# SmartBFT-Go/consensus

Measured on NVIDIA H100. Metric: ECDSA-P256 verifies/sec at batch=64K, higher is better.
Workload: dtype u32 limbs (integer)

## Files before the change

consensus_b200/csrc/inst_common.cuh:

```cuda
#pragma once
#include "keygroup.cuh"
#include "ops.h"
#include <cstdlib>

namespace sbv {

template <class C> struct Cfg;
template <> struct Cfg<P256> { static constexpr int COZ_MINB = 6, KT_MINB = 7, KT_VARIANT = 2, COMB_MINB = 6; static constexpr bool COMB_INL = true; };
template <> struct Cfg<P384> { static constexpr int COZ_MINB = 4, KT_MINB = 4, KT_VARIANT = 0; };

template <class C>
cudaError_t op_gtable_init(uint32_t *gtab, cudaStream_t st) {
    const size_t entries = (size_t)C::GWINS << C::GW;
    k_gtable_init<C><<<(unsigned)((entries + 127) / 128), 128, 0, st>>>(gtab);
    return cudaGetLastError();
}

template <class C>
cudaError_t op_prep(uint32_t n, const uint8_t *r, const uint8_t *s, const uint8_t *dig, uint32_t dlen, uint32_t *uw, uint8_t *flags,
                    cudaStream_t st) {
    return launch_prep<C, 8>(n, r, s, dig, dlen, uw, flags, st);
}

template <class C>
cudaError_t op_group(uint32_t n, const uint8_t *qx, const uint8_t *qy, uint32_t seed, uint32_t hmask, uint32_t *htab, uint32_t *rep,
                     uint32_t *kcnt, uint32_t threshold, uint32_t max_keys, int32_t *keyid, uint32_t *keylist, int32_t *item_kid,
                     uint32_t *klist, uint32_t *glist, uint32_t *counters, int route, cudaStream_t st) {
    const unsigned blocks = (n + 255) / 256;
    k_kg_insert<C><<<blocks, 256, 0, st>>>(n, qx, qy, seed, hmask, htab, rep, kcnt);
    k_kg_assign<<<blocks, 256, 0, st>>>(n, rep, kcnt, threshold, max_keys, keyid, keylist, counters);
    if (route) k_kg_route<<<blocks, 256, 0, st>>>(n, rep, keyid, item_kid, klist, glist, counters);
    return cudaGetLastError();
}

[[maybe_unused]] static cudaError_t op_route(uint32_t n, const uint32_t *rep, const int32_t *keyid, int32_t *item_kid, uint32_t *klist, uint32_t *glist,
                            uint32_t *counters, cudaStream_t st) {
    k_kg_route<<<(n + 255) / 256, 256, 0, st>>>(n, rep, keyid, item_kid, klist, glist, counters);
    return cudaGetLastError();
}

template <class C>
cudaError_t op_gpart(uint32_t n, const uint32_t *uw, const uint32_t *gtab, uint32_t *gacc, cudaStream_t st) {
    constexpr int BLOCK = 64;
    k_gpart<C, BLOCK, Cfg<C>::KT_MINB - 1><<<(n + BLOCK - 1) / BLOCK, BLOCK, 0, st>>>(n, uw, reinterpret_cast<const uint4 *>(gtab), gacc);
    return cudaGetLastError();
}

template <class C>
cudaError_t op_coz(uint32_t n, const uint8_t *qx, const uint8_t *qy, const uint8_t *r, const uint32_t *uw, const uint8_t *flags,
                   const uint32_t *gtab, uint32_t *tscr, uint8_t *ok, const uint32_t *list, const uint32_t *count, cudaStream_t st) {
    constexpr int BLOCK = 64;
    const size_t smem = (size_t)7 * 2 * C::N * 4 * BLOCK;
    k_verify_coz<C, BLOCK, Cfg<C>::COZ_MINB><<<(n + BLOCK - 1) / BLOCK, BLOCK, smem, st>>>(
        n, qx, qy, r, uw, flags, reinterpret_cast<const uint4 *>(gtab), tscr, ok, list, count);
    return cudaGetLastError();
}

template <class C, int W>
cudaError_t op_kt_build(const uint32_t *nkeys_ptr, uint32_t cap, const uint32_t *keylist, const uint8_t *qx, const uint8_t *qy,
                        uint32_t *bases, uint32_t *hs, uint32_t *ztop, uint32_t *pref, uint32_t *ktab, uint8_t *keyflags, cudaStream_t st) {
    using KT = KeyTab<32 * C::N, W>;
    const unsigned kb = (cap + 63) / 64;
    const unsigned wb = (unsigned)(((size_t)cap * KT::NWIN + 63) / 64);
    static const int bases_variant = getenv("SBV_KT_BASES") ? atoi(getenv("SBV_KT_BASES")) : 0;
    if (bases_variant == 2) k_kt_bases<C, KT, false><<<kb, 64, 0, st>>>(nkeys_ptr, cap, keylist, qx, qy, bases, keyflags);
    else if (bases_variant == 1) k_kt_bases<C, KT, true><<<kb, 64, 0, st>>>(nkeys_ptr, cap, keylist, qx, qy, bases, keyflags);
    else k_kt_bases4<C, KT><<<(unsigned)(((size_t)cap * 4 + 127) / 128), 128, 0, st>>>(nkeys_ptr, cap, keylist, qx, qy, bases, keyflags);
    k_kt_fill<C, W><<<wb, 64, 0, st>>>(nkeys_ptr, cap, bases, keyflags, hs, ztop, ktab);
    k_kt_inv<C, KT><<<kb, 64, 0, st>>>(nkeys_ptr, cap, keyflags, ztop, pref);
    k_kt_final<C, KT><<<wb, 64, 0, st>>>(nkeys_ptr, cap, bases, keyflags, hs, ztop, ktab);
    return cudaGetLastError();
}

template <class C, int W>
cudaError_t op_kt_verify(int reg, int warp, uint32_t n, const uint32_t *slot, const int32_t *kidmap, uint32_t n_slots,
                         const uint8_t *keyflags, const uint8_t *r, const uint32_t *uw, const uint8_t *flags, const uint32_t *gtab,
                         const uint32_t *ktab, uint8_t *ok, const uint32_t *list, const uint32_t *count, const uint32_t *gacc, cudaStream_t st) {
    constexpr int BLOCK = 64, MINB = Cfg<C>::KT_MINB;
    static const int variant = getenv("SBV_KT_VARIANT") ? atoi(getenv("SBV_KT_VARIANT")) : Cfg<C>::KT_VARIANT;
    const uint4 *g4 = reinterpret_cast<const uint4 *>(gtab), *k4 = reinterpret_cast<const uint4 *>(ktab);
    const unsigned blocks = (n + BLOCK - 1) / BLOCK;
#define SBV_KT_ARGS n, slot, kidmap, n_slots, keyflags, r, uw, flags, g4, k4, ok, list, count, gacc
    if (warp) {
        k_verify_kt_warp<C, W><<<(unsigned)(((size_t)n * 32 + 127) / 128), 128, 0, st>>>(n, slot, kidmap, n_slots, keyflags, r, uw, flags, g4, k4, ok);
    } else if (reg) {
        if (variant == 1) k_verify_kt<C, W, BLOCK, MINB, true, true><<<blocks, BLOCK, 0, st>>>(SBV_KT_ARGS);
        else if (variant == 2) k_verify_kt<C, W, BLOCK, MINB - 1, true, true><<<blocks, BLOCK, 0, st>>>(SBV_KT_ARGS);
        else k_verify_kt<C, W, BLOCK, MINB, true, false><<<blocks, BLOCK, 0, st>>>(SBV_KT_ARGS);
    } else {
        if (variant == 1) k_verify_kt<C, W, BLOCK, MINB, false, true><<<blocks, BLOCK, 0, st>>>(SBV_KT_ARGS);
        else if (variant == 2) k_verify_kt<C, W, BLOCK, MINB - 1, false, true><<<blocks, BLOCK, 0, st>>>(SBV_KT_ARGS);
        else k_verify_kt<C, W, BLOCK, MINB, false, false><<<blocks, BLOCK, 0, st>>>(SBV_KT_ARGS);
    }
#undef SBV_KT_ARGS
    return cudaGetLastError();
}

template <class C>
cudaError_t op_comb_build(const uint32_t *nkeys_ptr, uint32_t cap, const uint32_t *keylist, const uint8_t *qx, const uint8_t *qy,
                          uint32_t *bases, uint32_t *hs, uint32_t *ztop, uint32_t *pref, uint32_t *ktab, uint8_t *keyflags, cudaStream_t st) {
    using CT = CombTab<C>;
    const unsigned kb = (cap + 63) / 64;
    const unsigned cb = (unsigned)(((size_t)cap * CT::NCHAIN + 63) / 64);
    k_kt_bases4<C, CT><<<(unsigned)(((size_t)cap * 4 + 127) / 128), 128, 0, st>>>(nkeys_ptr, cap, keylist, qx, qy, bases, keyflags);
    k_comb_affine<C><<<kb, 64, 0, st>>>(nkeys_ptr, cap, keyflags, bases, pref);
    k_comb_fill<C><<<cb, 64, 0, st>>>(nkeys_ptr, cap, bases, keyflags, hs, ztop, ktab);
    k_kt_inv<C, CT><<<kb, 64, 0, st>>>(nkeys_ptr, cap, keyflags, ztop, pref);
    k_kt_final<C, CT><<<cb, 64, 0, st>>>(nkeys_ptr, cap, bases, keyflags, hs, ztop, ktab);
    return cudaGetLastError();
}

template <class C>
cudaError_t op_comb_verify(int reg, int warp, uint32_t n, const uint32_t *slot, const int32_t *kidmap, uint32_t n_slots,
                           const uint8_t *keyflags, const uint8_t *r, const uint32_t *uw, const uint8_t *flags, const uint32_t *gtab,
                           const uint32_t *ktab, uint8_t *ok, const uint32_t *list, const uint32_t *count, const uint32_t *gacc, cudaStream_t st) {
    constexpr int BLOCK = 64;
    (void)slot; (void)n_slots;
    if (reg || warp || !list || !count) return cudaErrorInvalidValue;
    k_verify_comb<C, BLOCK, Cfg<C>::COMB_MINB, Cfg<C>::COMB_INL><<<(n + BLOCK - 1) / BLOCK, BLOCK, 0, st>>>(
        n, kidmap, keyflags, r, uw, flags, reinterpret_cast<const uint4 *>(gtab), reinterpret_cast<const uint4 *>(ktab), ok, list, count, gacc);
    return cudaGetLastError();
}

template <class C, class KT>
constexpr KtGeom kt_geom() {
    using KS = KtSizes<C, KT>;
    return KtGeom{KS::bases_words(1), KS::hs_words(1), KS::ztop_words(1), KS::ktab_words(1)};
}

}
```

consensus_b200/csrc/keygroup.cuh:

```cuda
#pragma once
#include "kernels.cuh"

namespace sbv {

constexpr uint32_t KG_EMPTY = 0xffffffffu;

template <class C>
SBV_DEV uint32_t kg_hash(const uint8_t *__restrict__ qx_be, const uint8_t *__restrict__ qy_be, uint32_t i, uint32_t seed) {
    const uint32_t *x = reinterpret_cast<const uint32_t *>(qx_be + (size_t)i * C::BYTES);
    const uint32_t *y = reinterpret_cast<const uint32_t *>(qy_be + (size_t)i * C::BYTES);
    uint32_t h = seed;
#pragma unroll
    for (int k = 0; k < C::N; k += 2) {
        h = (h ^ __ldg(x + k)) * 0x9E3779B1u;
        h = (h ^ __ldg(y + k + 1)) * 0x85EBCA77u;
        h ^= h >> 15;
    }
    return h;
}
template <class C>
SBV_DEV bool kg_same_key(const uint8_t *__restrict__ qx_be, const uint8_t *__restrict__ qy_be, uint32_t i, uint32_t j) {
    const uint32_t *xi = reinterpret_cast<const uint32_t *>(qx_be + (size_t)i * C::BYTES);
    const uint32_t *xj = reinterpret_cast<const uint32_t *>(qx_be + (size_t)j * C::BYTES);
    const uint32_t *yi = reinterpret_cast<const uint32_t *>(qy_be + (size_t)i * C::BYTES);
    const uint32_t *yj = reinterpret_cast<const uint32_t *>(qy_be + (size_t)j * C::BYTES);
    uint32_t diff = 0;
#pragma unroll
    for (int k = 0; k < C::N; k++) diff |= (__ldg(xi + k) ^ __ldg(xj + k)) | (__ldg(yi + k) ^ __ldg(yj + k));
    return diff == 0;
}

template <class C>
__global__ void __launch_bounds__(256) k_kg_insert(uint32_t n, const uint8_t *__restrict__ qx_be, const uint8_t *__restrict__ qy_be,
                                                   uint32_t seed, uint32_t hmask, uint32_t *__restrict__ htab,
                                                   uint32_t *__restrict__ rep, uint32_t *__restrict__ kcnt) {
    const uint32_t i = blockIdx.x * blockDim.x + threadIdx.x;
    if (i >= n) return;
    uint32_t h = kg_hash<C>(qx_be, qy_be, i, seed) & hmask;
    uint32_t r;
    for (;;) {
        uint32_t cur = htab[h];
        if (cur == KG_EMPTY) {
            cur = atomicCAS(htab + h, KG_EMPTY, i);
            if (cur == KG_EMPTY) { r = i; break; }
        }
        if (kg_same_key<C>(qx_be, qy_be, i, cur)) { r = cur; break; }
        h = (h + 1) & hmask;
    }
    rep[i] = r;
#if defined(__CUDA_ARCH__)
    const uint32_t peers = __match_any_sync(__activemask(), r);
    if ((threadIdx.x & 31) == (uint32_t)(__ffs((int)peers) - 1)) atomicAdd(kcnt + r, (uint32_t)__popc(peers));
#else
    atomicAdd(kcnt + r, 1u);
#endif
}

static __global__ void __launch_bounds__(256) k_kg_assign(uint32_t n, const uint32_t *__restrict__ rep, const uint32_t *__restrict__ kcnt,
                                                   uint32_t threshold, uint32_t max_keys, int32_t *__restrict__ keyid,
                                                   uint32_t *__restrict__ keylist, uint32_t *__restrict__ counters) {
    const uint32_t i = blockIdx.x * blockDim.x + threadIdx.x;
    if (i >= n) return;
    int32_t id = -1;
    if (rep[i] == i && kcnt[i] >= threshold) {
        const uint32_t k = atomicAdd(counters + 0, 1u);
        if (k < max_keys) { id = (int32_t)k; keylist[k] = i; }
    }
    keyid[i] = id;
}

static __global__ void __launch_bounds__(256) k_kg_route(uint32_t n, const uint32_t *__restrict__ rep, const int32_t *__restrict__ keyid,
                                                  int32_t *__restrict__ item_kid, uint32_t *__restrict__ klist, uint32_t *__restrict__ glist,
                                                  uint32_t *__restrict__ counters) {
    const uint32_t i = blockIdx.x * blockDim.x + threadIdx.x;
    const bool live = i < n;
    const int32_t kid = live ? keyid[rep[i]] : -1;
    if (live) item_kid[i] = kid;
#if defined(__CUDA_ARCH__)
    const uint32_t lane = threadIdx.x & 31;
    const uint32_t mk = __ballot_sync(0xffffffffu, live && kid >= 0), mg = __ballot_sync(0xffffffffu, live && kid < 0);
    uint32_t bk = 0, bg = 0;
    if (lane == 0) {
        if (mk) bk = atomicAdd(counters + 1, (uint32_t)__popc(mk));
        if (mg) bg = atomicAdd(counters + 2, (uint32_t)__popc(mg));
    }
    bk = __shfl_sync(0xffffffffu, bk, 0);
    bg = __shfl_sync(0xffffffffu, bg, 0);
    const uint32_t below = (1u << lane) - 1u;
    if (live && kid >= 0) klist[bk + __popc(mk & below)] = i;
    if (live && kid < 0) glist[bg + __popc(mg & below)] = i;
#else
    if (live && kid >= 0) klist[atomicAdd(counters + 1, 1u)] = i;
    if (live && kid < 0) glist[atomicAdd(counters + 2, 1u)] = i;
#endif
}


template <class C, class KT, bool INL>
__global__ void __launch_bounds__(64) k_kt_bases(const uint32_t *__restrict__ nkeys_ptr, uint32_t cap, const uint32_t *__restrict__ keylist,
                                                 const uint8_t *__restrict__ qx_be, const uint8_t *__restrict__ qy_be,
                                                 uint32_t *__restrict__ bases, uint8_t *__restrict__ keyflags) {
    constexpr int N = C::N;
    const uint32_t k = blockIdx.x * blockDim.x + threadIdx.x;
    uint32_t nkeys = __ldg(nkeys_ptr);
    if (nkeys > cap) nkeys = cap;
    if (k >= nkeys) return;
    const uint32_t item = keylist ? keylist[k] : k;
    using A = typename PickArith<C, INL>::type;
    Jac<A> B;
    const bool good = load_key<C>(B.X, B.Y, qx_be, qy_be, item);
    keyflags[k] = good ? 1 : 0;
    if (!good) return;
    C::get_one(B.Z);
#pragma unroll 1
    for (int win = 0; win < KT::NBASE; win++) {
        if (win) {
#pragma unroll 1
            for (int d = 0; d < KT::STEP; d++) pt_double<A>(B);
        }
        uint32_t *o = bases + (size_t)win * 3 * N * cap + k;
#pragma unroll
        for (int i = 0; i < N; i++) { o[(size_t)i * cap] = B.X[i]; o[(size_t)(N + i) * cap] = B.Y[i]; o[(size_t)(2 * N + i) * cap] = B.Z[i]; }
    }
}

template <class C, class KT>
__global__ void __launch_bounds__(128) k_kt_bases4(const uint32_t *__restrict__ nkeys_ptr, uint32_t cap, const uint32_t *__restrict__ keylist,
                                                   const uint8_t *__restrict__ qx_be, const uint8_t *__restrict__ qy_be,
                                                   uint32_t *__restrict__ bases, uint8_t *__restrict__ keyflags) {
    constexpr int N = C::N;
    const uint32_t gt = blockIdx.x * blockDim.x + threadIdx.x;
    const uint32_t k = gt >> 2, role = gt & 3;
    uint32_t nkeys = __ldg(nkeys_ptr);
    if (nkeys > cap) nkeys = cap;
    if (k >= nkeys) return;
    const unsigned qbase = (threadIdx.x & 31) & ~3u, qmask = 0xFu << qbase;
    const uint32_t item = keylist ? keylist[k] : k;
    uint32_t X[N], Y[N], Z[N];
    const bool good = load_key<C>(X, Y, qx_be, qy_be, item);
    if (role == 0) keyflags[k] = good ? 1 : 0;
    if (!good) return;
    C::get_one(Z);
    auto bcast = [&](uint32_t (&v)[N], unsigned src) {
#pragma unroll
        for (int i = 0; i < N; i++) v[i] = __shfl_sync(qmask, v[i], qbase + src);
    };
#pragma unroll 1
    for (int win = 0; win < KT::NBASE; win++) {
        if (win) {
#pragma unroll 1
            for (int d = 0; d < KT::STEP; d++) {
                uint32_t s[N], a[N], b[N], r1[N], r2[N], r3[N], r4[N], t1[N], t2[N];
                C::fadd(s, Y, Y);
                mp_select<N>(a, role == 1 || role == 2, s, Z);
                mp_select<N>(b, role == 1, s, Z);
                C::fmul(r1, a, b);
                uint32_t bb[N];
                mp_copy<N>(bb, r1);
                bcast(bb, 1);
                C::fsub(t1, X, r1);
                C::fadd(t2, X, r1);
                mp_select<N>(a, role == 0, t1, X);
                mp_select<N>(a, role == 2, bb, a);
                mp_select<N>(b, role == 0, t2, bb);
                C::fmul(r2, a, b);
                uint32_t alpha[N], half[N], beta4[N];
                C::fadd(t1, r2, r2);
                C::fadd(alpha, t1, r2);
                C::fhalf(half, r2);
                C::fmul(r3, alpha, alpha);
                mp_copy<N>(beta4, r2);
                bcast(beta4, 1);
                bcast(half, 2);
                uint32_t x3[N], y3[N];
                C::fadd(t1, beta4, beta4);
                C::fsub(x3, r3, t1);
                C::fsub(t2, beta4, x3);
                C::fmul(r4, alpha, t2);
                C::fsub(y3, r4, half);
                mp_copy<N>(X, x3); bcast(X, 0);
                mp_copy<N>(Y, y3); bcast(Y, 0);
                mp_copy<N>(Z, r1); bcast(Z, 2);
            }
        }
        if (role == 0) {
            uint32_t *o = bases + (size_t)win * 3 * N * cap + k;
#pragma unroll
            for (int i = 0; i < N; i++) { o[(size_t)i * cap] = X[i]; o[(size_t)(N + i) * cap] = Y[i]; o[(size_t)(2 * N + i) * cap] = Z[i]; }
        }
    }
}

template <class C>
SBV_DEV void zaddu(uint32_t (&X1)[C::N], uint32_t (&Y1)[C::N], const uint32_t (&X2)[C::N], const uint32_t (&Y2)[C::N],
                   uint32_t (&X3)[C::N], uint32_t (&Y3)[C::N], uint32_t (&h)[C::N]) {
    constexpr int N = C::N;
    uint32_t c[N], w1[N], w2[N], dy[N], d[N], a1[N], t[N];
    C::fsub(h, X1, X2);
    C::fsqr(c, h);
    C::fmul(w1, X1, c);
    C::fmul(w2, X2, c);
    C::fsub(dy, Y1, Y2);
    C::fsqr(d, dy);
    C::fsub(t, w1, w2);
    C::fmul(a1, Y1, t);
    C::fsub(X3, d, w1);
    C::fsub(X3, X3, w2);
    C::fsub(t, w1, X3);
    C::fmul(Y3, dy, t);
    C::fsub(Y3, Y3, a1);
    mp_copy<N>(X1, w1);
    mp_copy<N>(Y1, a1);
}

template <class C, int W>
__global__ void __launch_bounds__(64) k_kt_fill(const uint32_t *__restrict__ nkeys_ptr, uint32_t cap, const uint32_t *__restrict__ bases,
                                                const uint8_t *__restrict__ keyflags, uint32_t *__restrict__ hs,
                                                uint32_t *__restrict__ ztop, uint32_t *__restrict__ ktab) {
    constexpr int N = C::N;
    using KT = KeyTab<32 * N, W>;
    const uint32_t t = blockIdx.x * blockDim.x + threadIdx.x;
    uint32_t nkeys = __ldg(nkeys_ptr);
    if (nkeys > cap) nkeys = cap;
    if (t >= nkeys * KT::NWIN) return;
    const uint32_t k = t % nkeys, win = t / nkeys;
    if (!keyflags[k]) return;
    uint32_t bx[N], by[N], bz[N];
    {
        const uint32_t *o = bases + (size_t)win * 3 * N * cap + k;
#pragma unroll
        for (int i = 0; i < N; i++) { bx[i] = o[(size_t)i * cap]; by[i] = o[(size_t)(N + i) * cap]; bz[i] = o[(size_t)(2 * N + i) * cap]; }
    }
    uint32_t *out = ktab + ((size_t)k * KT::NWIN + win) * KT::ENT * 2 * N;
#pragma unroll
    for (int i = 0; i < N; i++) { out[i] = bx[i]; out[N + i] = by[i]; }
    Jac<C> P;
    mp_copy<N>(P.X, bx); mp_copy<N>(P.Y, by); mp_copy<N>(P.Z, bz);
    uint32_t h[N], h2[N], h3[N];
    C::fadd(h, by, by);
    pt_double<C>(P);
    C::fsqr(h2, h);
    C::fmul(h3, h2, h);
    C::fmul(bx, bx, h2);
    C::fmul(by, by, h3);
    uint32_t zacc[N];
    mp_copy<N>(zacc, P.Z);
    {
        uint32_t *hp = hs + ((size_t)win * (KT::ENT - 1) + 0) * N * cap + k;
#pragma unroll
        for (int i = 0; i < N; i++) { out[2 * N + i] = P.X[i]; out[3 * N + i] = P.Y[i]; hp[(size_t)i * cap] = h[i]; }
    }
    uint32_t px[N], py[N];
    mp_copy<N>(px, P.X); mp_copy<N>(py, P.Y);
#pragma unroll 1
    for (int e = 3; e <= KT::ENT; e++) {
        uint32_t x3[N], y3[N];
        zaddu<C>(bx, by, px, py, x3, y3, h);
        C::fmul(zacc, zacc, h);
        mp_copy<N>(px, x3); mp_copy<N>(py, y3);
        uint32_t *hp = hs + ((size_t)win * (KT::ENT - 1) + (e - 2)) * N * cap + k;
        uint32_t *oe = out + (size_t)(e - 1) * 2 * N;
#pragma unroll
        for (int i = 0; i < N; i++) { oe[i] = px[i]; oe[N + i] = py[i]; hp[(size_t)i * cap] = h[i]; }
    }
    uint32_t *zp = ztop + (size_t)win * N * cap + k;
#pragma unroll
    for (int i = 0; i < N; i++) zp[(size_t)i * cap] = zacc[i];
}

template <class C, class KT>
__global__ void __launch_bounds__(64) k_kt_inv(const uint32_t *__restrict__ nkeys_ptr, uint32_t cap, const uint8_t *__restrict__ keyflags,
                                               uint32_t *__restrict__ ztop, uint32_t *__restrict__ pref) {
    constexpr int N = C::N;
    const uint32_t k = blockIdx.x * blockDim.x + threadIdx.x;
    uint32_t nkeys = __ldg(nkeys_ptr);
    if (nkeys > cap) nkeys = cap;
    if (k >= nkeys || !keyflags[k]) return;
    uint32_t run[N];
    C::get_one(run);
#pragma unroll 1
    for (int win = 0; win < KT::NCHAIN; win++) {
        uint32_t z[N];
        const uint32_t *zp = ztop + (size_t)win * N * cap + k;
        uint32_t *pp = pref + (size_t)win * N * cap + k;
#pragma unroll
        for (int i = 0; i < N; i++) { z[i] = zp[(size_t)i * cap]; pp[(size_t)i * cap] = run[i]; }
        C::fmul(run, run, z);
    }
    uint32_t inv[N];
    p_inv<C>(inv, run);
#pragma unroll 1
    for (int win = KT::NCHAIN - 1; win >= 0; win--) {
        uint32_t z[N], pv[N], zi[N];
        uint32_t *zp = ztop + (size_t)win * N * cap + k;
        const uint32_t *pp = pref + (size_t)win * N * cap + k;
#pragma unroll
        for (int i = 0; i < N; i++) { z[i] = zp[(size_t)i * cap]; pv[i] = pp[(size_t)i * cap]; }
        C::fmul(zi, inv, pv);
        C::fmul(inv, inv, z);
#pragma unroll
        for (int i = 0; i < N; i++) zp[(size_t)i * cap] = zi[i];
    }
}

template <class C, class KT>
__global__ void __launch_bounds__(64) k_kt_final(const uint32_t *__restrict__ nkeys_ptr, uint32_t cap, const uint32_t *__restrict__ bases,
                                                 const uint8_t *__restrict__ keyflags, const uint32_t *__restrict__ hs,
                                                 const uint32_t *__restrict__ ztop, uint32_t *__restrict__ ktab) {
    constexpr int N = C::N;
    const uint32_t t = blockIdx.x * blockDim.x + threadIdx.x;
    uint32_t nkeys = __ldg(nkeys_ptr);
    if (nkeys > cap) nkeys = cap;
    if (t >= nkeys * KT::NCHAIN) return;
    const uint32_t k = t % nkeys, win = t / nkeys;
    if (!keyflags[k]) return;
    uint32_t zi[N];
    {
        const uint32_t *zp = ztop + (size_t)win * N * cap + k;
#pragma unroll
        for (int i = 0; i < N; i++) zi[i] = zp[(size_t)i * cap];
    }
    uint32_t *out = ktab + ((size_t)k * KT::NCHAIN + win) * KT::ENT * 2 * N;
    uint32_t x[N], y[N], h[N];
    {
        const uint32_t *oe = out + (size_t)(KT::ENT - 1) * 2 * N;
#pragma unroll
        for (int i = 0; i < N; i++) { x[i] = oe[i]; y[i] = oe[N + i]; }
    }
#pragma unroll 1
    for (int e = KT::ENT; e >= 1; e--) {
        uint32_t nx[N], ny[N], nh[N];
        if (e >= 2) {
            const uint32_t *on = out + (size_t)(e - 2) * 2 * N;
            const uint32_t *hp = hs + ((size_t)win * (KT::ENT - 1) + (e - 2)) * N * cap + k;
#pragma unroll
            for (int i = 0; i < N; i++) { nx[i] = on[i]; ny[i] = on[N + i]; nh[i] = hp[(size_t)i * cap]; }
        }
        uint32_t *oe = out + (size_t)(e - 1) * 2 * N;
        uint32_t z2[N], z3[N];
        C::fsqr(z2, zi);
        C::fmul(z3, z2, zi);
        C::fmul(x, x, z2);
        C::fmul(y, y, z3);
#pragma unroll
        for (int i = 0; i < N; i++) { oe[i] = x[i]; oe[N + i] = y[i]; }
        if (e >= 2) {
            mp_copy<N>(h, nh);
            C::fmul(zi, zi, h);
            mp_copy<N>(x, nx); mp_copy<N>(y, ny);
        }
    }
    (void)bases;
}


template <class C>
__global__ void __launch_bounds__(64) k_comb_affine(const uint32_t *__restrict__ nkeys_ptr, uint32_t cap, const uint8_t *__restrict__ keyflags,
                                                    uint32_t *__restrict__ bases, uint32_t *__restrict__ pref) {
    constexpr int N = C::N;
    using CT = CombTab<C>;
    const uint32_t k = blockIdx.x * blockDim.x + threadIdx.x;
    uint32_t nkeys = __ldg(nkeys_ptr);
    if (nkeys > cap) nkeys = cap;
    if (k >= nkeys || !keyflags[k]) return;
    uint32_t run[N];
    C::get_one(run);
#pragma unroll 1
    for (int c = 0; c < CT::NBASE; c++) {
        uint32_t z[N];
        const uint32_t *zp = bases + ((size_t)c * 3 + 2) * N * cap + k;
        uint32_t *pp = pref + (size_t)c * N * cap + k;
#pragma unroll
        for (int i = 0; i < N; i++) { z[i] = zp[(size_t)i * cap]; pp[(size_t)i * cap] = run[i]; }
        C::fmul(run, run, z);
    }
    uint32_t inv[N];
    p_inv<C>(inv, run);
#pragma unroll 1
    for (int c = CT::NBASE - 1; c >= 0; c--) {
        uint32_t *o = bases + (size_t)c * 3 * N * cap + k;
        const uint32_t *pp = pref + (size_t)c * N * cap + k;
        uint32_t x[N], y[N], z[N], pv[N], zi[N], z2[N], z3[N];
#pragma unroll
        for (int i = 0; i < N; i++) { x[i] = o[(size_t)i * cap]; y[i] = o[(size_t)(N + i) * cap]; z[i] = o[(size_t)(2 * N + i) * cap]; pv[i] = pp[(size_t)i * cap]; }
        C::fmul(zi, inv, pv);
        C::fmul(inv, inv, z);
        C::fsqr(z2, zi);
        C::fmul(z3, z2, zi);
        C::fmul(x, x, z2);
        C::fmul(y, y, z3);
#pragma unroll
        for (int i = 0; i < N; i++) { o[(size_t)i * cap] = x[i]; o[(size_t)(N + i) * cap] = y[i]; }
    }
}

template <class C>
__global__ void __launch_bounds__(64) k_comb_fill(const uint32_t *__restrict__ nkeys_ptr, uint32_t cap, const uint32_t *__restrict__ bases,
                                                  const uint8_t *__restrict__ keyflags, uint32_t *__restrict__ hs,
                                                  uint32_t *__restrict__ ztop, uint32_t *__restrict__ ktab) {
    constexpr int N = C::N;
    using CT = CombTab<C>;
    const uint32_t t = blockIdx.x * blockDim.x + threadIdx.x;
    uint32_t nkeys = __ldg(nkeys_ptr);
    if (nkeys > cap) nkeys = cap;
    if (t >= nkeys * CT::NCHAIN) return;
    const uint32_t k = t % nkeys, ch = t / nkeys;
    if (!keyflags[k]) return;
    const int b = (int)(ch >> 4), hi = (int)(ch & 15);
    auto base = [&](int c, uint32_t (&x)[N], uint32_t (&y)[N]) {
        const uint32_t *o = bases + (size_t)c * 3 * N * cap + k;
#pragma unroll
        for (int i = 0; i < N; i++) { x[i] = o[(size_t)i * cap]; y[i] = o[(size_t)(N + i) * cap]; }
    };
    uint32_t *out = ktab + ((size_t)k * CT::NCHAIN + ch) * CT::ENT * 2 * N;
    auto store = [&](int slot, const uint32_t (&x)[N], const uint32_t (&y)[N], const uint32_t (&h)[N]) {
        uint32_t *o = out + (size_t)slot * 2 * N;
#pragma unroll
        for (int i = 0; i < N; i++) { o[i] = x[i]; o[N + i] = y[i]; }
        if (slot) {
            uint32_t *hp = hs + ((size_t)ch * (CT::ENT - 1) + (slot - 1)) * N * cap + k;
#pragma unroll
            for (int i = 0; i < N; i++) hp[(size_t)i * cap] = h[i];
        }
    };
    Jac<C> P;
    uint32_t x[N], y[N], h[N];
    C::get_one(P.Z);
    C::get_one(h);
    int first;
    if (hi == 0) {
        uint32_t zero[N];
#pragma unroll
        for (int i = 0; i < N; i++) zero[i] = 0;
        store(0, zero, zero, h);
        base(CT::TEETH * b, P.X, P.Y);
        store(1, P.X, P.Y, h);
        first = 2;
    } else {
        bool empty = true;
#pragma unroll 1
        for (int i = 0; i < 4; i++) {
            if (!((hi >> i) & 1)) continue;
            base(CT::TEETH * b + 4 + i, x, y);
            if (empty) { mp_copy<N>(P.X, x); mp_copy<N>(P.Y, y); empty = false; }
            else pt_madd_table<C>(P, x, y, h);
        }
        store(0, P.X, P.Y, h);
        first = 1;
    }
#pragma unroll 1
    for (int kk = first; kk < CT::ENT; kk++) {
        const int tooth = __ffs(kk) - 1;
        base(CT::TEETH * b + tooth, x, y);
        if (!(((kk ^ (kk >> 1)) >> tooth) & 1)) {
            uint32_t zero[N];
#pragma unroll
            for (int i = 0; i < N; i++) zero[i] = 0;
            C::fsub(y, zero, y);
        }
        pt_madd_table<C>(P, x, y, h);
        store(kk, P.X, P.Y, h);
    }
    uint32_t *zp = ztop + (size_t)ch * N * cap + k;
#pragma unroll
    for (int i = 0; i < N; i++) zp[(size_t)i * cap] = P.Z[i];
}

template <class C, class KT_>
struct KtSizes {
    using KT = KT_;
    static constexpr size_t bases_words(size_t cap) { return (size_t)KT::NBASE * 3 * C::N * cap; }
    static constexpr size_t hs_words(size_t cap) { return (size_t)KT::NCHAIN * (KT::ENT - 1) * C::N * cap; }
    static constexpr size_t ztop_words(size_t cap) { return (size_t)KT::NCHAIN * C::N * cap; }
    static constexpr size_t ktab_words(size_t cap) { return KT::POINTS * 2 * C::N * cap; }
};

}
```

consensus_b200/csrc/pipeline.cu:

```cuda
#include "engine.h"

namespace {

int take_scratch(sbv_engine *e, Dev &d, const CurveOps &ops, const KtOps *kt, size_t n, size_t kcap, cudaStream_t st, Dev::Scratch **out) {
    int idx = (int)(d.ws_next++ % SBV_SCRATCH);
    for (int tries = 0; tries < SBV_SCRATCH && d.ws[idx].open; tries++) idx = (int)(d.ws_next++ % SBV_SCRATCH);
    if (d.ws[idx].open) return sbv_fail(e, SBV_ERR_ARG, "no free scratch set (more launches held open than lanes?)");
    Dev::Scratch &w = d.ws[idx];
    Dev::Scratch::Caps &c = w.caps;
    if (!w.done) {
        for (int j = 0; j < SBV_SCRATCH; j++) {
            Dev::Scratch &x = d.ws[j];
            if (x.done) continue;
            CU(e, cudaEventCreateWithFlags(&x.done, cudaEventDisableTiming));
            CU(e, cudaEventCreateWithFlags(&x.ev_group, cudaEventDisableTiming));
            CU(e, cudaEventCreateWithFlags(&x.ev_prep, cudaEventDisableTiming));
            CU(e, cudaEventCreateWithFlags(&x.ev_tab, cudaEventDisableTiming));
            CU(e, cudaEventCreateWithFlags(&x.ev_gen, cudaEventDisableTiming));
            if (e->tab_hi) {
                int lo_p = 0, hi_p = 0;
                CU(e, cudaDeviceGetStreamPriorityRange(&lo_p, &hi_p));
                CU(e, cudaStreamCreateWithPriority(&x.s_tab, cudaStreamNonBlocking, hi_p));
            } else {
                CU(e, cudaStreamCreateWithFlags(&x.s_tab, cudaStreamNonBlocking));
            }
            CU(e, cudaStreamCreateWithFlags(&x.s_gen, cudaStreamNonBlocking));
        }
    }
    const size_t N = (size_t)ops.N;
    uint32_t hsize = 1;
    while (hsize < 2 * n) hsize <<= 1;
    struct Need { void **p; size_t *cap; size_t need, alloc; };
    const size_t ni = n + n / 8 + 1024, kc = kcap + kcap / 8 + 16;
    uint32_t hs2 = 1;
    while (hs2 < 2 * ni) hs2 <<= 1;
    const bool g = kcap > 0, t = g && kt;
    const KtGeom z{};
    const KtGeom &q = t ? kt->geom : z;
    Need needs[] = {
        {(void **)&w.uw, &c.uw, 2 * N * n * 4, 2 * N * ni * 4},
        {(void **)&w.flags, &c.flags, n, ni},
        {(void **)&w.tscr, &c.tscr, 12 * N * n * 4, 12 * N * ni * 4},
        {(void **)&w.gacc, &c.gacc, g ? 3 * N * n * 4 : 0, 3 * N * ni * 4},
        {(void **)&w.htab, &c.htab, g ? (size_t)hsize * 4 : 0, (size_t)hs2 * 4},
        {(void **)&w.rep, &c.rep, g ? n * 4 : 0, ni * 4},
        {(void **)&w.klist, &c.klist, g ? n * 4 : 0, ni * 4},
        {(void **)&w.glist, &c.glist, g ? n * 4 : 0, ni * 4},
        {(void **)&w.zeroed, &c.zeroed, g ? (n + 4 + 4 * SBV_MAX_CHUNKS) * 4 : 0, (ni + 4 + 4 * SBV_MAX_CHUNKS) * 4},
        {(void **)&w.keyid, &c.keyid, g ? n * 4 : 0, ni * 4},
        {(void **)&w.item_kid, &c.item_kid, g ? n * 4 : 0, ni * 4},
        {(void **)&w.keylist, &c.keylist, t ? kcap * 4 : 0, kc * 4},
        {(void **)&w.keyflags, &c.keyflags, t ? kcap : 0, kc},
        {(void **)&w.bases, &c.bases, q.bases_words * kcap * 4, q.bases_words * kc * 4},
        {(void **)&w.hs, &c.hs, q.hs_words * kcap * 4, q.hs_words * kc * 4},
        {(void **)&w.ztop, &c.ztop, q.ztop_words * kcap * 4, q.ztop_words * kc * 4},
        {(void **)&w.pref, &c.pref, q.ztop_words * kcap * 4, q.ztop_words * kc * 4},
        {(void **)&w.ktab, &c.ktab, q.ktab_words * kcap * 4, q.ktab_words * kc * 4},
    };
    bool grows = false;
    for (const Need &nd : needs) grows = grows || nd.need > *nd.cap;
    if (grows) {
        for (int j = 0; j < SBV_SCRATCH; j++) {
            Dev::Scratch &x = d.ws[j];
            if (x.open && &x != &w) continue;
            if (x.used && x.done) CU(e, cudaEventSynchronize(x.done));
            Dev::Scratch::Caps &cx = x.caps;
            struct Slot { void **p; size_t *cap; };
            const Slot slots[] = {
                {(void **)&x.uw, &cx.uw}, {(void **)&x.flags, &cx.flags}, {(void **)&x.tscr, &cx.tscr}, {(void **)&x.gacc, &cx.gacc},
                {(void **)&x.htab, &cx.htab}, {(void **)&x.rep, &cx.rep}, {(void **)&x.klist, &cx.klist}, {(void **)&x.glist, &cx.glist},
                {(void **)&x.zeroed, &cx.zeroed}, {(void **)&x.keyid, &cx.keyid}, {(void **)&x.item_kid, &cx.item_kid}, {(void **)&x.keylist, &cx.keylist},
                {(void **)&x.keyflags, &cx.keyflags}, {(void **)&x.bases, &cx.bases}, {(void **)&x.hs, &cx.hs}, {(void **)&x.ztop, &cx.ztop},
                {(void **)&x.pref, &cx.pref}, {(void **)&x.ktab, &cx.ktab},
            };
            static_assert(sizeof(slots) / sizeof(slots[0]) == sizeof(needs) / sizeof(needs[0]), "one slot per buffer");
            for (size_t q = 0; q < sizeof(slots) / sizeof(slots[0]); q++) {
                if (needs[q].need <= *slots[q].cap) continue;
                if (*slots[q].p) cudaFree(*slots[q].p);
                *slots[q].p = nullptr;
                *slots[q].cap = 0;
                CU(e, cudaMalloc(slots[q].p, needs[q].alloc));
                *slots[q].cap = needs[q].alloc;
            }
        }
    }
    w.hsize = hsize;
    if (w.used) CU(e, cudaStreamWaitEvent(st, w.done, 0));
    w.used = true;
    *out = &w;
    return 0;
}

cudaEvent_t *prof_take(sbv_engine *e, Dev &d) {
    if (!e->profiling) return nullptr;
    if (d.prof_used + 5 > d.prof_events.size()) {
        size_t old = d.prof_events.size();
        d.prof_events.resize(old + 128);
        for (size_t i = old; i < d.prof_events.size(); i++)
            if (cudaEventCreate(&d.prof_events[i]) != cudaSuccess) { d.prof_events.resize(i); return nullptr; }
    }
    cudaEvent_t *ev = &d.prof_events[d.prof_used];
    d.prof_used += 5;
    return ev;
}

}

void sbv_scratch_free(Dev &d) {
    for (auto &w : d.ws) {
        void *ptrs[] = {w.uw, w.flags, w.tscr, w.gacc, w.htab, w.rep, w.keylist, w.klist, w.glist, w.zeroed, w.keyid, w.item_kid, w.bases, w.hs, w.ztop, w.pref, w.ktab, w.keyflags};
        for (void *p : ptrs) if (p) cudaFree(p);
        cudaEvent_t evs[] = {w.done, w.ev_group, w.ev_prep, w.ev_tab, w.ev_gen};
        for (cudaEvent_t ev : evs) if (ev) cudaEventDestroy(ev);
        if (w.s_tab) cudaStreamDestroy(w.s_tab);
        if (w.s_gen) cudaStreamDestroy(w.s_gen);
        w = Dev::Scratch{};
    }
}

int sbv_init_gtables(sbv_engine *e, Dev &d) {
    for (int c = 0; c < 2; c++) {
        const CurveOps &ops = sbv_ops(c);
        CU(e, cudaMalloc(&d.gtab[c], ops.gtab_entries * 2 * ops.N * 4));
        CU(e, ops.gtable_init(d.gtab[c], d.stream));
    }
    e->launches += 2;
    CU(e, cudaStreamSynchronize(d.stream));
    return 0;
}

int sbv_launch_verify_begin(sbv_engine *e, Dev &d, uint8_t curve, size_t n, const uint8_t *d_qx, const uint8_t *d_qy, cudaStream_t st,
                            VerifyLaunch *vl, int chunks) {
    *vl = VerifyLaunch{};
    if (n == 0) return 0;
    if (chunks < 1 || chunks > SBV_MAX_CHUNKS) return sbv_fail(e, SBV_ERR_ARG, "bad chunk count %d", chunks);
    const CurveOps &ops = sbv_ops(curve);
    const KtOps *kt = ops.grouped;
    const uint32_t nn = (uint32_t)n;
    const uint32_t T = e->group_threshold > 0 ? (uint32_t)e->group_threshold : 0;
    const bool grouping = T > 0 && n >= T && n >= (size_t)e->group_min_batch && e->group_max_keys > 0;
    size_t kcap = 0;
    if (grouping) {
        kcap = n / T;
        if (kcap > (size_t)e->group_max_keys) kcap = (size_t)e->group_max_keys;
        if (kcap == 0) kcap = 1;
    }
    Dev::Scratch *w = nullptr;
    if (int rc = take_scratch(e, d, ops, grouping ? kt : nullptr, n, kcap, st, &w)) return rc;
    w->open = true;
    vl->w = w; vl->curve = curve; vl->n = n; vl->grouping = grouping; vl->d_qx = d_qx; vl->d_qy = d_qy; vl->chunks = chunks;
    vl->ev = prof_take(e, d);
    if (vl->ev) CU(e, cudaEventRecord(vl->ev[0], st));
    if (!grouping) return 0;
    uint32_t *counters = w->zeroed, *kcnt = w->zeroed + 4;
    CU(e, cudaMemsetAsync(w->htab, 0xff, (size_t)w->hsize * 4, st));
    CU(e, cudaMemsetAsync(w->zeroed, 0, (n + 4 + (chunks > 1 ? 4 * chunks : 0)) * 4, st));
    CU(e, ops.group(nn, d_qx, d_qy, e->hash_seed, w->hsize - 1, w->htab, w->rep, kcnt, T, (uint32_t)kcap, w->keyid, w->keylist, w->item_kid, w->klist,
                    w->glist, counters, chunks == 1, st));
    CU(e, cudaEventRecord(w->ev_group, st));
    CU(e, cudaStreamWaitEvent(w->s_tab, w->ev_group, 0));
    CU(e, kt->build(counters + 0, (uint32_t)kcap, w->keylist, d_qx, d_qy, w->bases, w->hs, w->ztop, w->pref, w->ktab, w->keyflags, w->s_tab));
    CU(e, cudaEventRecord(w->ev_tab, w->s_tab));
    e->launches += (chunks == 1 ? 3 : 2) + (curve == 0 ? 5 : 4);
    return 0;
}

int sbv_launch_verify_chunk(sbv_engine *e, Dev &d, const VerifyLaunch &vl, int c, size_t lo, size_t cn, bool last, const uint8_t *d_r, const uint8_t *d_s,
                            const uint8_t *d_dig, uint32_t dlen, uint8_t *d_ok, cudaStream_t st) {
    if (vl.n == 0) return 0;
    Dev::Scratch *w = vl.w;
    if (vl.chunks <= 1 || c < 0 || c >= vl.chunks || lo + cn > vl.n) return sbv_fail(e, SBV_ERR_ARG, "bad chunk");
    const CurveOps &ops = sbv_ops(vl.curve);
    const KtOps *kt = ops.grouped;
    const size_t N = (size_t)ops.N, L = (size_t)ops.bytes;
    const uint32_t nn = (uint32_t)cn;
    const uint32_t *gtab = d.gtab[vl.curve];
    cudaEvent_t *ev = last ? vl.ev : nullptr;
    if (ev) CU(e, cudaEventRecord(ev[0], st));
    uint32_t *uw = w->uw + 2 * N * lo, *tscr = w->tscr + 12 * N * lo;
    uint8_t *flags = w->flags + lo;
    const uint8_t *r = d_r + lo * L;
    if (cn) {
        CU(e, ops.prep(nn, r, d_s + lo * L, d_dig + lo * dlen, dlen, uw, flags, st));
        e->launches += 1;
    }
    if (ev) CU(e, cudaEventRecord(ev[1], st));
    if (!vl.grouping) {
        if (ev) { CU(e, cudaEventRecord(ev[4], st)); CU(e, cudaEventRecord(ev[2], st)); }
        if (cn) {
            CU(e, ops.coz(nn, vl.d_qx + lo * L, vl.d_qy + lo * L, r, uw, flags, gtab, tscr, d_ok + lo, nullptr, nullptr, st));
            e->launches += 1;
        }
        if (ev) CU(e, cudaEventRecord(ev[3], st));
    } else if (cn) {
        uint32_t *cc = w->zeroed + 4 + vl.n + 4 * (size_t)c;
        uint32_t *klist = w->klist + lo, *glist = w->glist + lo;
        CU(e, ops.route(nn, w->rep + lo, w->keyid, w->item_kid + lo, klist, glist, cc, st));
        CU(e, cudaEventRecord(w->ev_prep, st));
        CU(e, cudaStreamWaitEvent(w->s_gen, w->ev_prep, 0));
        CU(e, ops.coz(nn, vl.d_qx + lo * L, vl.d_qy + lo * L, r, uw, flags, gtab, tscr, d_ok + lo, glist, cc + 2, w->s_gen));
        CU(e, cudaEventRecord(w->ev_gen, w->s_gen));
        const uint32_t *gacc = nullptr;
        if (e->gsplit) {
            uint32_t *ga = w->gacc + 3 * N * lo;
            CU(e, ops.gpart(nn, uw, gtab, ga, st));
            gacc = ga;
            e->launches += 1;
        }
        if (ev) CU(e, cudaEventRecord(ev[4], st));
        if (c == 0) CU(e, cudaStreamWaitEvent(st, w->ev_tab, 0));
        if (ev) CU(e, cudaEventRecord(ev[2], st));
        CU(e, kt->verify(0, 0, nn, nullptr, w->item_kid + lo, 0, w->keyflags, r, uw, flags, gtab, w->ktab, d_ok + lo, klist, cc + 1, gacc, st));
        if (ev) CU(e, cudaEventRecord(ev[3], st));
        CU(e, cudaStreamWaitEvent(st, w->ev_gen, 0));
        e->launches += 3;
    } else if (ev) {
        CU(e, cudaEventRecord(ev[4], st)); CU(e, cudaEventRecord(ev[2], st)); CU(e, cudaEventRecord(ev[3], st));
    }
    if (last) {
        CU(e, cudaEventRecord(w->done, st));
        w->open = false;
    }
    return 0;
}

void sbv_launch_verify_abort(const VerifyLaunch &vl, cudaStream_t st) {
    Dev::Scratch *w = vl.w;
    if (!w || !w->open) return;
    if (vl.grouping) cudaStreamWaitEvent(st, w->ev_tab, 0);
    cudaStreamWaitEvent(st, w->ev_gen, 0);
    cudaEventRecord(w->done, st);
    w->open = false;
}

int sbv_launch_verify_finish(sbv_engine *e, Dev &d, const VerifyLaunch &vl, const uint8_t *d_r, const uint8_t *d_s, const uint8_t *d_dig,
                             uint32_t dlen, uint8_t *d_ok, cudaStream_t st) {
    if (vl.n == 0) return 0;
    if (vl.chunks != 1) return sbv_fail(e, SBV_ERR_ARG, "chunked launch finished in one piece");
    const CurveOps &ops = sbv_ops(vl.curve);
    const KtOps *kt = ops.grouped;
    Dev::Scratch *w = vl.w;
    cudaEvent_t *ev = vl.ev;
    const uint32_t nn = (uint32_t)vl.n;
    const uint32_t *gtab = d.gtab[vl.curve];
    CU(e, ops.prep(nn, d_r, d_s, d_dig, dlen, w->uw, w->flags, st));
    if (!vl.grouping) {
        if (ev) { CU(e, cudaEventRecord(ev[1], st)); CU(e, cudaEventRecord(ev[4], st)); CU(e, cudaEventRecord(ev[2], st)); }
        CU(e, ops.coz(nn, vl.d_qx, vl.d_qy, d_r, w->uw, w->flags, gtab, w->tscr, d_ok, nullptr, nullptr, st));
        if (ev) CU(e, cudaEventRecord(ev[3], st));
        CU(e, cudaEventRecord(w->done, st));
        w->open = false;
        e->launches += 2;
        return 0;
    }
    uint32_t *counters = w->zeroed;
    CU(e, cudaEventRecord(w->ev_prep, st));
    if (ev) CU(e, cudaEventRecord(ev[1], st));
    CU(e, cudaStreamWaitEvent(w->s_gen, w->ev_prep, 0));
    CU(e, ops.coz(nn, vl.d_qx, vl.d_qy, d_r, w->uw, w->flags, gtab, w->tscr, d_ok, w->glist, counters + 2, w->s_gen));
    CU(e, cudaEventRecord(w->ev_gen, w->s_gen));
    const uint32_t *gacc = nullptr;
    if (e->gsplit) {
        CU(e, ops.gpart(nn, w->uw, gtab, w->gacc, st));
        gacc = w->gacc;
        e->launches += 1;
    }
    if (ev) CU(e, cudaEventRecord(ev[4], st));
    CU(e, cudaStreamWaitEvent(st, w->ev_tab, 0));
    if (ev) CU(e, cudaEventRecord(ev[2], st));
    CU(e, kt->verify(0, 0, nn, nullptr, w->item_kid, 0, w->keyflags, d_r, w->uw, w->flags, gtab, w->ktab, d_ok, w->klist, counters + 1, gacc, st));
    if (ev) CU(e, cudaEventRecord(ev[3], st));
    CU(e, cudaStreamWaitEvent(st, w->ev_gen, 0));
    CU(e, cudaEventRecord(w->done, st));
    w->open = false;
    e->launches += 3;
    return 0;
}

int sbv_launch_verify(sbv_engine *e, Dev &d, uint8_t curve, size_t n, const uint8_t *d_r, const uint8_t *d_s, const uint8_t *d_qx,
                      const uint8_t *d_qy, const uint8_t *d_dig, uint32_t dlen, uint8_t *d_ok, cudaStream_t st) {
    VerifyLaunch vl;
    if (int rc = sbv_launch_verify_begin(e, d, curve, n, d_qx, d_qy, st, &vl)) return rc;
    return sbv_launch_verify_finish(e, d, vl, d_r, d_s, d_dig, dlen, d_ok, st);
}

void sbv_keys_free(Dev &d) {
    for (int c = 0; c < 2; c++) {
        if (d.ktab[c]) cudaFree(d.ktab[c]);
        if (d.keyflags[c]) cudaFree(d.keyflags[c]);
        if (d.slot2local[c]) cudaFree(d.slot2local[c]);
        d.ktab[c] = nullptr; d.keyflags[c] = nullptr; d.slot2local[c] = nullptr; d.n_local[c] = 0;
    }
    d.n_slots = 0;
}

int sbv_keys_build(sbv_engine *e, Dev &d) {
    CU(e, cudaSetDevice(d.ordinal));
    CU(e, cudaDeviceSynchronize());
    sbv_keys_free(d);
    const size_t n = e->key_ids.size();
    d.n_slots = (uint32_t)n;
    if (n == 0) return 0;
    for (int c = 0; c < 2; c++) {
        const CurveOps &ops = sbv_ops(c);
        const KtOps *kt = ops.kt8;
        const size_t L = (size_t)ops.bytes;
        std::vector<int32_t> map(n, -1);
        std::vector<uint8_t> kx, ky;
        uint32_t cnt = 0;
        for (size_t i = 0; i < n; i++) {
            if (e->key_curve[i] != c) continue;
            const uint8_t *x = &e->key_xy[96 * i], *y = x + 48;
            bool fits = true;
            for (size_t b = 0; b < 48 - L; b++) if (x[b] || y[b]) fits = false;
            if (!fits) continue;
            map[i] = (int32_t)cnt++;
            kx.insert(kx.end(), x + (48 - L), x + 48);
            ky.insert(ky.end(), y + (48 - L), y + 48);
        }
        CU(e, cudaMalloc(&d.slot2local[c], n * sizeof(int32_t)));
        CU(e, cudaMemcpyAsync(d.slot2local[c], map.data(), n * sizeof(int32_t), cudaMemcpyHostToDevice, d.stream));
        d.n_local[c] = cnt;
        if (cnt == 0) { CU(e, cudaStreamSynchronize(d.stream)); continue; }
        CU(e, cudaMalloc(&d.ktab[c], kt->geom.ktab_words * cnt * 4));
        CU(e, cudaMalloc(&d.keyflags[c], cnt));
        uint8_t *d_kx = nullptr, *d_ky = nullptr;
        uint32_t *tmp = nullptr, *d_cnt = nullptr;
        const size_t tmp_words = (kt->geom.bases_words + kt->geom.hs_words + 2 * kt->geom.ztop_words) * cnt;
        CU(e, cudaMalloc(&d_kx, kx.size()));
        CU(e, cudaMalloc(&d_ky, ky.size()));
        CU(e, cudaMalloc(&tmp, tmp_words * 4));
        CU(e, cudaMalloc(&d_cnt, 4));
        CU(e, cudaMemcpyAsync(d_kx, kx.data(), kx.size(), cudaMemcpyHostToDevice, d.stream));
        CU(e, cudaMemcpyAsync(d_ky, ky.data(), ky.size(), cudaMemcpyHostToDevice, d.stream));
        CU(e, cudaMemcpyAsync(d_cnt, &cnt, 4, cudaMemcpyHostToDevice, d.stream));
        uint32_t *bases = tmp, *hs = bases + kt->geom.bases_words * cnt, *ztop = hs + kt->geom.hs_words * cnt, *pref = ztop + kt->geom.ztop_words * cnt;
        cudaError_t st = kt->build(d_cnt, cnt, nullptr, d_kx, d_ky, bases, hs, ztop, pref, d.ktab[c], d.keyflags[c], d.stream);
        e->launches += 4;
        if (st == cudaSuccess) st = cudaStreamSynchronize(d.stream);
        cudaFree(d_kx); cudaFree(d_ky); cudaFree(tmp); cudaFree(d_cnt);
        CU(e, st);
    }
    return 0;
}

int sbv_launch_keyed(sbv_engine *e, Dev &d, uint8_t curve, size_t n, const uint32_t *d_slot, const uint8_t *d_r, const uint8_t *d_s,
                     const uint8_t *d_dig, uint32_t dlen, uint8_t *d_ok, cudaStream_t st) {
    if (n == 0) return 0;
    if (d.n_local[curve] == 0) {
        CU(e, cudaMemsetAsync(d_ok, 0, n, st));
        return 0;
    }
    const CurveOps &ops = sbv_ops(curve);
    const KtOps *kt = ops.kt8;
    const uint32_t nn = (uint32_t)n;
    Dev::Scratch *w = nullptr;
    if (int rc = take_scratch(e, d, ops, nullptr, n, 0, st, &w)) return rc;
    cudaEvent_t *ev = prof_take(e, d);
    if (ev) CU(e, cudaEventRecord(ev[0], st));
    CU(e, ops.prep(nn, d_r, d_s, d_dig, dlen, w->uw, w->flags, st));
    if (ev) { CU(e, cudaEventRecord(ev[1], st)); CU(e, cudaEventRecord(ev[4], st)); CU(e, cudaEventRecord(ev[2], st)); }
    const int warp = nn <= (uint32_t)e->keyed_warp_limit ? 1 : 0;
    CU(e, kt->verify(1, warp, nn, d_slot, d.slot2local[curve], d.n_slots, d.keyflags[curve], d_r, w->uw, w->flags, d.gtab[curve], d.ktab[curve], d_ok,
                     nullptr, nullptr, nullptr, st));
    if (ev) CU(e, cudaEventRecord(ev[3], st));
    CU(e, cudaEventRecord(w->done, st));
    e->launches += 2;
    return 0;
}
```

Measured before the change: 67.93 million.

## Replace comb base affine inversion with common-Z normalization fused into bases kernel

Removes the separate k_comb_affine kernel, which inverted the product of base Z coordinates per key to convert the comb bases to affine. Instead, the bases kernel rescales all bases to a shared Z coordinate via prefix products, with the 4-lane variant combining partial products through warp shuffles. The common Z is then folded into the chain Z in comb_fill, so no per-key field inversion or extra launch is needed. Window stores are spread across the four lanes. The cost is extra multiplications and global traffic inside the bases kernel.

```diff
diff --git a/consensus_b200/csrc/inst_common.cuh b/consensus_b200/csrc/inst_common.cuh
--- a/consensus_b200/csrc/inst_common.cuh
+++ b/consensus_b200/csrc/inst_common.cuh
@@ -63,9 +63,9 @@
     const unsigned kb = (cap + 63) / 64;
     const unsigned wb = (unsigned)(((size_t)cap * KT::NWIN + 63) / 64);
     static const int bases_variant = getenv("SBV_KT_BASES") ? atoi(getenv("SBV_KT_BASES")) : 0;
-    if (bases_variant == 2) k_kt_bases<C, KT, false><<<kb, 64, 0, st>>>(nkeys_ptr, cap, keylist, qx, qy, bases, keyflags);
-    else if (bases_variant == 1) k_kt_bases<C, KT, true><<<kb, 64, 0, st>>>(nkeys_ptr, cap, keylist, qx, qy, bases, keyflags);
-    else k_kt_bases4<C, KT><<<(unsigned)(((size_t)cap * 4 + 127) / 128), 128, 0, st>>>(nkeys_ptr, cap, keylist, qx, qy, bases, keyflags);
+    if (bases_variant == 2) k_kt_bases<C, KT, false><<<kb, 64, 0, st>>>(nkeys_ptr, cap, keylist, qx, qy, bases, pref, keyflags);
+    else if (bases_variant == 1) k_kt_bases<C, KT, true><<<kb, 64, 0, st>>>(nkeys_ptr, cap, keylist, qx, qy, bases, pref, keyflags);
+    else k_kt_bases4<C, KT><<<(unsigned)(((size_t)cap * 4 + 127) / 128), 128, 0, st>>>(nkeys_ptr, cap, keylist, qx, qy, bases, pref, keyflags);
     k_kt_fill<C, W><<<wb, 64, 0, st>>>(nkeys_ptr, cap, bases, keyflags, hs, ztop, ktab);
     k_kt_inv<C, KT><<<kb, 64, 0, st>>>(nkeys_ptr, cap, keyflags, ztop, pref);
     k_kt_final<C, KT><<<wb, 64, 0, st>>>(nkeys_ptr, cap, bases, keyflags, hs, ztop, ktab);
@@ -102,8 +102,7 @@
     using CT = CombTab<C>;
     const unsigned kb = (cap + 63) / 64;
     const unsigned cb = (unsigned)(((size_t)cap * CT::NCHAIN + 63) / 64);
-    k_kt_bases4<C, CT><<<(unsigned)(((size_t)cap * 4 + 127) / 128), 128, 0, st>>>(nkeys_ptr, cap, keylist, qx, qy, bases, keyflags);
-    k_comb_affine<C><<<kb, 64, 0, st>>>(nkeys_ptr, cap, keyflags, bases, pref);
+    k_kt_bases4<C, CT><<<(unsigned)(((size_t)cap * 4 + 127) / 128), 128, 0, st>>>(nkeys_ptr, cap, keylist, qx, qy, bases, pref, keyflags);
     k_comb_fill<C><<<cb, 64, 0, st>>>(nkeys_ptr, cap, bases, keyflags, hs, ztop, ktab);
     k_kt_inv<C, CT><<<kb, 64, 0, st>>>(nkeys_ptr, cap, keyflags, ztop, pref);
     k_kt_final<C, CT><<<cb, 64, 0, st>>>(nkeys_ptr, cap, bases, keyflags, hs, ztop, ktab);
diff --git a/consensus_b200/csrc/keygroup.cuh b/consensus_b200/csrc/keygroup.cuh
--- a/consensus_b200/csrc/keygroup.cuh
+++ b/consensus_b200/csrc/keygroup.cuh
@@ -1,4 +1,6 @@
 #pragma once
+#include <type_traits>
+
 #include "kernels.cuh"
 
 namespace sbv {
@@ -96,10 +98,61 @@
 }
 
 
+template <class C, int LANES, class Others>
+SBV_DEV void comb_common_z(uint32_t *__restrict__ bases, uint32_t *__restrict__ pref, uint32_t cap, uint32_t k, uint32_t lane,
+                           Others &&others) {
+    constexpr int N = C::N, J = CombTab<C>::NBASE / LANES;
+    static_assert(J * LANES == CombTab<C>::NBASE, "every lane owns the same number of bases");
+    auto zslot = [&](int j) { return bases + ((size_t)(LANES * j + lane) * 3 + 2) * N * cap + k; };
+    auto pslot = [&](int j) { return pref + (size_t)(LANES * j + lane) * N * cap + k; };
+    uint32_t run[N], s[N];
+    C::get_one(run);
+#pragma unroll 1
+    for (int j = 0; j < J; j++) {
+        const uint32_t *zo = zslot(j);
+        uint32_t *po = pslot(j);
+        uint32_t z[N];
+#pragma unroll
+        for (int i = 0; i < N; i++) { z[i] = zo[(size_t)i * cap]; po[(size_t)i * cap] = run[i]; }
+        C::fmul(run, run, z);
+    }
+    others(s, run);
+#pragma unroll 1
+    for (int j = J - 1; j >= 0; j--) {
+        uint32_t *o = bases + (size_t)(LANES * j + lane) * 3 * N * cap + k;
+        const uint32_t *zo = zslot(j), *po = pslot(j);
+        uint32_t v[N], lam[N], l2[N];
+#pragma unroll
+        for (int i = 0; i < N; i++) lam[i] = po[(size_t)i * cap];
+        C::fmul(lam, lam, s);
+#pragma unroll
+        for (int i = 0; i < N; i++) v[i] = zo[(size_t)i * cap];
+        C::fmul(s, s, v);
+        C::fsqr(l2, lam);
+#pragma unroll
+        for (int i = 0; i < N; i++) v[i] = o[(size_t)i * cap];
+        C::fmul(v, v, l2);
+#pragma unroll
+        for (int i = 0; i < N; i++) o[(size_t)i * cap] = v[i];
+        C::fmul(l2, l2, lam);
+#pragma unroll
+        for (int i = 0; i < N; i++) v[i] = o[(size_t)(N + i) * cap];
+        C::fmul(v, v, l2);
+#pragma unroll
+        for (int i = 0; i < N; i++) o[(size_t)(N + i) * cap] = v[i];
+    }
+#pragma unroll 1
+    for (int j = 0; j < J; j++) {
+        uint32_t *o = bases + ((size_t)(LANES * j + lane) * 3 + 2) * N * cap + k;
+#pragma unroll
+        for (int i = 0; i < N; i++) o[(size_t)i * cap] = s[i];
+    }
+}
+
 template <class C, class KT, bool INL>
 __global__ void __launch_bounds__(64) k_kt_bases(const uint32_t *__restrict__ nkeys_ptr, uint32_t cap, const uint32_t *__restrict__ keylist,
                                                  const uint8_t *__restrict__ qx_be, const uint8_t *__restrict__ qy_be,
-                                                 uint32_t *__restrict__ bases, uint8_t *__restrict__ keyflags) {
+                                                 uint32_t *__restrict__ bases, uint32_t *__restrict__ pref, uint8_t *__restrict__ keyflags) {
     constexpr int N = C::N;
     const uint32_t k = blockIdx.x * blockDim.x + threadIdx.x;
     uint32_t nkeys = __ldg(nkeys_ptr);
@@ -122,12 +175,13 @@
 #pragma unroll
         for (int i = 0; i < N; i++) { o[(size_t)i * cap] = B.X[i]; o[(size_t)(N + i) * cap] = B.Y[i]; o[(size_t)(2 * N + i) * cap] = B.Z[i]; }
     }
+    if constexpr (std::is_same<KT, CombTab<C>>::value) comb_common_z<C, 1>(bases, pref, cap, k, 0, [](uint32_t (&s)[N], const uint32_t (&)[N]) { C::get_one(s); });
 }
 
 template <class C, class KT>
 __global__ void __launch_bounds__(128) k_kt_bases4(const uint32_t *__restrict__ nkeys_ptr, uint32_t cap, const uint32_t *__restrict__ keylist,
                                                    const uint8_t *__restrict__ qx_be, const uint8_t *__restrict__ qy_be,
-                                                   uint32_t *__restrict__ bases, uint8_t *__restrict__ keyflags) {
+                                                   uint32_t *__restrict__ bases, uint32_t *__restrict__ pref, uint8_t *__restrict__ keyflags) {
     constexpr int N = C::N;
     const uint32_t gt = blockIdx.x * blockDim.x + threadIdx.x;
     const uint32_t k = gt >> 2, role = gt & 3;
@@ -183,11 +237,25 @@
                 mp_copy<N>(Z, r1); bcast(Z, 2);
             }
         }
-        if (role == 0) {
+        if ((uint32_t)(win & 3) == role) {
             uint32_t *o = bases + (size_t)win * 3 * N * cap + k;
 #pragma unroll
             for (int i = 0; i < N; i++) { o[(size_t)i * cap] = X[i]; o[(size_t)(N + i) * cap] = Y[i]; o[(size_t)(2 * N + i) * cap] = Z[i]; }
         }
+    }
+    if constexpr (std::is_same<KT, CombTab<C>>::value) {
+        comb_common_z<C, 4>(bases, pref, cap, k, role, [&](uint32_t (&s)[N], const uint32_t (&run)[N]) {
+            uint32_t a[N];
+#pragma unroll
+            for (int i = 0; i < N; i++) {
+                s[i] = __shfl_sync(qmask, run[i], qbase + (role ^ 1));
+                a[i] = __shfl_sync(qmask, run[i], qbase + (role ^ 2));
+            }
+            C::fmul(s, s, a);
+#pragma unroll
+            for (int i = 0; i < N; i++) a[i] = __shfl_sync(qmask, run[i], qbase + (role ^ 3));
+            C::fmul(s, s, a);
+        });
     }
 }
 
@@ -355,46 +423,6 @@
 
 
 template <class C>
-__global__ void __launch_bounds__(64) k_comb_affine(const uint32_t *__restrict__ nkeys_ptr, uint32_t cap, const uint8_t *__restrict__ keyflags,
-                                                    uint32_t *__restrict__ bases, uint32_t *__restrict__ pref) {
-    constexpr int N = C::N;
-    using CT = CombTab<C>;
-    const uint32_t k = blockIdx.x * blockDim.x + threadIdx.x;
-    uint32_t nkeys = __ldg(nkeys_ptr);
-    if (nkeys > cap) nkeys = cap;
-    if (k >= nkeys || !keyflags[k]) return;
-    uint32_t run[N];
-    C::get_one(run);
-#pragma unroll 1
-    for (int c = 0; c < CT::NBASE; c++) {
-        uint32_t z[N];
-        const uint32_t *zp = bases + ((size_t)c * 3 + 2) * N * cap + k;
-        uint32_t *pp = pref + (size_t)c * N * cap + k;
-#pragma unroll
-        for (int i = 0; i < N; i++) { z[i] = zp[(size_t)i * cap]; pp[(size_t)i * cap] = run[i]; }
-        C::fmul(run, run, z);
-    }
-    uint32_t inv[N];
-    p_inv<C>(inv, run);
-#pragma unroll 1
-    for (int c = CT::NBASE - 1; c >= 0; c--) {
-        uint32_t *o = bases + (size_t)c * 3 * N * cap + k;
-        const uint32_t *pp = pref + (size_t)c * N * cap + k;
-        uint32_t x[N], y[N], z[N], pv[N], zi[N], z2[N], z3[N];
-#pragma unroll
-        for (int i = 0; i < N; i++) { x[i] = o[(size_t)i * cap]; y[i] = o[(size_t)(N + i) * cap]; z[i] = o[(size_t)(2 * N + i) * cap]; pv[i] = pp[(size_t)i * cap]; }
-        C::fmul(zi, inv, pv);
-        C::fmul(inv, inv, z);
-        C::fsqr(z2, zi);
-        C::fmul(z3, z2, zi);
-        C::fmul(x, x, z2);
-        C::fmul(y, y, z3);
-#pragma unroll
-        for (int i = 0; i < N; i++) { o[(size_t)i * cap] = x[i]; o[(size_t)(N + i) * cap] = y[i]; }
-    }
-}
-
-template <class C>
 __global__ void __launch_bounds__(64) k_comb_fill(const uint32_t *__restrict__ nkeys_ptr, uint32_t cap, const uint32_t *__restrict__ bases,
                                                   const uint8_t *__restrict__ keyflags, uint32_t *__restrict__ hs,
                                                   uint32_t *__restrict__ ztop, uint32_t *__restrict__ ktab) {
@@ -461,6 +489,13 @@
         pt_madd_table<C>(P, x, y, h);
         store(kk, P.X, P.Y, h);
     }
+    uint32_t zc[N];
+    {
+        const uint32_t *o = bases + (size_t)2 * N * cap + k;
+#pragma unroll
+        for (int i = 0; i < N; i++) zc[i] = o[(size_t)i * cap];
+    }
+    C::fmul(P.Z, P.Z, zc);
     uint32_t *zp = ztop + (size_t)ch * N * cap + k;
 #pragma unroll
     for (int i = 0; i < N; i++) zp[(size_t)i * cap] = P.Z[i];
diff --git a/consensus_b200/csrc/pipeline.cu b/consensus_b200/csrc/pipeline.cu
--- a/consensus_b200/csrc/pipeline.cu
+++ b/consensus_b200/csrc/pipeline.cu
@@ -161,7 +161,7 @@
     CU(e, cudaStreamWaitEvent(w->s_tab, w->ev_group, 0));
     CU(e, kt->build(counters + 0, (uint32_t)kcap, w->keylist, d_qx, d_qy, w->bases, w->hs, w->ztop, w->pref, w->ktab, w->keyflags, w->s_tab));
     CU(e, cudaEventRecord(w->ev_tab, w->s_tab));
-    e->launches += (chunks == 1 ? 3 : 2) + (curve == 0 ? 5 : 4);
+    e->launches += (chunks == 1 ? 3 : 2) + 4;
     return 0;
 }
 
```

Result: no change. 69.05 million (median of 6 runs) (+1.6%).
